# apache/cassandra

Hardware: NVIDIA H100
Metric: compaction MB/s (uncompressed in) (higher is better)
Workload: dtype u8

## Files before the change

cassandra_b200/csrc/codec.cuh:

```cuda
#pragma once
#include "common.cuh"
#include "lz4.cuh"
#include "lz4_chain.cuh"
#include "snappy_chain.cuh"
#include "snappy.cuh"
#include "codec_defs.cuh"
#include "lz4_thread.cuh"
#include "lz4_batch.cuh"

namespace b200c {

__global__ void __launch_bounds__(32) k_compress_chunks(const DevTables* __restrict__ T, int comp, int tab_bytes,
        const uint8_t* __restrict__ in, uint64_t n, int chunk_len, int max_clen,
        uint8_t* __restrict__ slots, int slot_stride, uint32_t* __restrict__ file_len, uint32_t* __restrict__ seg_raw) {
    extern __shared__ __align__(16) uint8_t smem[];
    uint16_t* s_tab = (uint16_t*)smem;
    uint8_t* s_in = smem + tab_bytes;
    const int lane = threadIdx.x;
    const uint64_t chunk = blockIdx.x;
    const uint64_t start = chunk * (uint64_t)chunk_len;
    const int ulen = (int)min((uint64_t)chunk_len, n - start);
    const uint8_t* src = in + start;

    if ((((uintptr_t)src) & 15) == 0) {
// ... 412 lines not shown
}

enum : uint32_t { K1_SKIP = 0xFFFFFFFFu, K1_BAD = 0xFFFFFFFEu, K1_BAD_OFFS = 0xFFFFFFFDu, K1_RAW = 0xFFFFFFFCu };
struct K1Chunk { const uint8_t* src; uint8_t* dst; int clen, ulen; uint64_t slot, ctag; };
__device__ __forceinline__ uint32_t k1_locate(const K1Seg* __restrict__ segs, int nseg, uint64_t t, K1Chunk& k) {
    int lo = 0, hi = nseg - 1;
    while (lo < hi) { int mid = (lo + hi + 1) >> 1; if (segs[mid].first <= t) lo = mid; else hi = mid - 1; }
    const K1Seg& g = segs[lo];
    const uint64_t chunk = g.chunk0 + (t - g.first);
    if (chunk >= g.nchunks) return K1_SKIP;
    const uint64_t off = g.offs[chunk], next = (chunk + 1 < g.nchunks) ? g.offs[chunk + 1] : g.data_len, off0 = g.offs[g.chunk0];
    const uint64_t ustart = chunk * (uint64_t)g.chunk_len;
    k.ctag = ((uint64_t)g.tag << 40) | chunk;
    if (off + 4 > next || next > g.data_len || ustart >= g.data_length || next - off - 4 > (uint64_t)(chunk_max_compressed(COMP_LZ4, g.chunk_len) + g.chunk_len) ||
        off < off0 || next - off0 > g.rec_span) return K1_BAD_OFFS;
    k.clen = (int)(next - off - 4); k.ulen = (int)min((uint64_t)g.chunk_len, g.data_length - ustart);
    k.src = k1_src(g.data, g.tail, g.tail_off, off); k.dst = g.out + ustart;
    k.slot = g.rec0 + (off - off0) / 3 + 2 * (chunk - g.chunk0);
    return k.clen >= g.max_clen ? K1_RAW : 0u;
}
__global__ void __launch_bounds__(128) k_lz4_walk_multi(const K1Seg* __restrict__ segs, int nseg, uint64_t total, uint16_t* __restrict__ rec,
                                                        uint32_t* __restrict__ nseq, ChunkErr* __restrict__ err) {
    const uint64_t t = (uint64_t)blockIdx.x * blockDim.x + threadIdx.x;
    if (t >= total) return;
    K1Chunk k; const uint32_t st = k1_locate(segs, nseg, t, k);
    if (st == K1_SKIP) { nseq[t] = K1_SKIP; return; }
    if (st == K1_BAD_OFFS) { report_chunk_err(err, k.ctag, 2); nseq[t] = K1_BAD_OFFS; return; }
    if (st == K1_RAW) { if (k.clen < k.ulen) { report_chunk_err(err, k.ctag, 2); nseq[t] = K1_BAD; } else nseq[t] = K1_RAW; return; }
    const uint8_t* src = k.src;
    const int plen = (k.clen >= 4) ? (int)((uint32_t)src[0] | ((uint32_t)src[1] << 8) | ((uint32_t)src[2] << 16) | ((uint32_t)src[3] << 24)) : -1;
    const int r = (plen == k.ulen) ? lz4_walk_thread(src + 4, k.clen - 4, k.ulen, rec + k.slot, (k.clen + 4) / 3 + 1) : -1;
    if (r < 0) { report_chunk_err(err, k.ctag, 2); nseq[t] = K1_BAD; } else nseq[t] = (uint32_t)r;
}
enum { K1C_WARPS = 4 };
__global__ void __launch_bounds__(32 * K1C_WARPS) k_lz4_copy_multi(const DevTables* __restrict__ T, const K1Seg* __restrict__ segs, int nseg, uint64_t total,
                                                                   const uint16_t* __restrict__ rec, const uint32_t* __restrict__ nseq, int verify, ChunkErr* __restrict__ err) {
    const int lane = threadIdx.x & 31;
    const uint64_t t = (uint64_t)blockIdx.x * K1C_WARPS + (threadIdx.x >> 5);
    if (t >= total) return;
    const uint32_t ns = nseq[t];
    if (ns == K1_SKIP || ns == K1_BAD_OFFS) return;
    K1Chunk k; (void)k1_locate(segs, nseg, t, k);
    if (verify) {
        const uint32_t crc = warp_crc32(T, T->crc_adv128, k.src, k.clen, lane);
        const uint8_t* s = k.src + k.clen;
        const uint32_t stored = ((uint32_t)s[0] << 24) | ((uint32_t)s[1] << 16) | ((uint32_t)s[2] << 8) | s[3];
        if (crc != stored) { if (lane == 0) report_chunk_err(err, k.ctag, 1); return; }
    }
    if (ns == K1_BAD) return;
    if (ns == K1_RAW) { for (int i = lane; i < k.ulen; i += 32) k.dst[i] = k.src[i]; return; }
    (void)lz4_copy_warp(k.src + 4, k.clen - 4, rec + k.slot, (int)ns, k.dst, lane);
}

}
```

cassandra_b200/csrc/engine.cu:

```cuda
#include "engine.cuh"
#include <algorithm>
#include "scan.cuh"
#include "codec.cuh"
#include <climits>
#include <vector>

using namespace b200c;

namespace b200c {

enum { WSC_IN = 0, WSC_OUT, WSC_SLOTS, WSC_FILELEN, WSC_SEGRAW, WSC_OFFS, WSC_ACC, WSC_ERR, WSC_CHOFFS, WSC_SCAN0, WSC_SCAN1, WSC_SCAN2 };
int raw_chunks_device(b200c_ctx* c, bool ingest, const RawArgs& a);
static int raw_digest(b200c_ctx* c, const uint32_t* seg_raw, const uint64_t* ends, uint64_t nchunks, uint32_t* acc, uint32_t* digest);

static void build_tables(DevTables* t) {
    for (uint32_t i = 0; i < 256; i++) {
        uint32_t c = i;
        for (int k = 0; k < 8; k++) c = (c & 1) ? (0xEDB88320u ^ (c >> 1)) : (c >> 1);
        t->crc_t[0][i] = c;
    }
    for (uint32_t i = 0; i < 256; i++)
        for (int k = 1; k < 4; k++) t->crc_t[k][i] = (t->crc_t[k - 1][i] >> 8) ^ t->crc_t[0][t->crc_t[k - 1][i] & 0xff];
    uint32_t sq = 0x00800000u;
    for (int k = 0; k < 64; k++) { t->xp_pow2[k] = sq; sq = gf2_mulmod(sq, sq); }
// ... 177 lines not shown
    b200c_ctx* c = o.c;
    *out_len = 0; *digest = 0; *d_offs_out = nullptr;
    if (!o.nchunks) return B200C_OK;
    if (o.raw) {
        B200C_TRY(raw_digest(c, o.seg_raw, o.ends, o.nchunks, o.acc, digest));
        B200C_CUDA_TRY(c, cudaStreamSynchronize(c->copy_out));
        *out_len = o.ulen; *d_offs_out = o.d_offs;
        return B200C_OK;
    }
    uint32_t* h32 = &c->h_pinned->os_digest;
    B200C_LAUNCH(c, k_digest, (unsigned)((o.nchunks + 255) / 256), 256, 0, c->d_tables, o.seg_raw, o.d_offs, o.nchunks, o.acc);
    B200C_LAUNCH(c, k_digest_final, 1, 1, 0, c->d_tables, o.d_offs, o.nchunks, o.acc);
    B200C_CUDA_TRY(c, cudaMemcpyAsync(h32, o.acc + 1, 4, cudaMemcpyDeviceToHost, c->stream));
    B200C_TRY(out_stream_drain(o, o.piece - 1));
    B200C_CUDA_TRY(c, cudaStreamSynchronize(c->stream));
    B200C_CUDA_TRY(c, cudaStreamSynchronize(c->copy_out));
    *out_len = o.copied; *digest = h32[0]; *d_offs_out = o.d_offs;
    return B200C_OK;
}

static void k1_plan(b200c_ctx* c) {
    static const int carveout_kb[] = {0, 8, 16, 32, 64, 100, 132, 164, 196, 228};
    const int per_sm = (int)std::max<uint64_t>(1, (uint64_t)c->l2_bytes / K1_L2_BYTES_PER_CHAIN / K1_THREADS / (uint64_t)c->nsm);
    const int block = c->smem_reserved_per_block + K1_STATIC_SMEM;
    int carve = c->smem_per_sm;
    for (int kb : carveout_kb) if (kb * 1024 >= per_sm * block) { carve = std::min(kb * 1024, c->smem_per_sm); break; }
    c->k1_blocks_per_sm = per_sm;
    c->k1_smem = (size_t)std::max(0, (carve / per_sm - block) & ~127);
    for (const void* k : {(const void*)k_decompress_multi_thr, (const void*)k_decompress_chunks_thr}) {
        cudaFuncSetAttribute(k, cudaFuncAttributeMaxDynamicSharedMemorySize, (int)c->k1_smem);
        cudaFuncSetAttribute(k, cudaFuncAttributePreferredSharedMemoryCarveout, 100 * carve / c->smem_per_sm);
    }
}
static unsigned k1_grid(const b200c_ctx* c, uint64_t nthreads) {
    return (unsigned)std::min<uint64_t>((uint64_t)c->k1_blocks_per_sm * (uint64_t)c->nsm, (nthreads + K1_THREADS - 1) / K1_THREADS);
}

int decompress_stream_device(b200c_ctx* c, int comp, const uint8_t* d_data, uint64_t data_len, const uint64_t* d_offs, uint64_t nchunks,
                             int chunk_len, int max_clen, uint64_t data_length, uint8_t* d_out, int verify, ChunkErr* d_err,
                             uint64_t chunk0, uint64_t count, int tag, const uint8_t* tail, uint64_t tail_off) {
    if (chunk0 >= nchunks || count == 0) return B200C_OK;
    const uint64_t end = count > nchunks - chunk0 ? nchunks : chunk0 + count;
    static const int k1_mode = []() { const char* e = getenv("B200C_K1"); return e ? atoi(e) : 1; }();
    if (k1_mode == 1 && comp == COMP_LZ4 && (chunk_len & 7) == 0 && ((uintptr_t)d_out & 7) == 0 && end - chunk0 >= 32768)
        B200C_LAUNCH(c, k_decompress_chunks_thr, k1_grid(c, end - chunk0), K1_THREADS, c->k1_smem, c->d_tables, comp, d_data, data_len, d_offs, nchunks,
                     chunk_len, max_clen, data_length, d_out, verify, d_err, chunk0, end, tag, tail, tail_off);
    else
        B200C_LAUNCH(c, k_decompress_chunks, (unsigned)((end - chunk0 + 1) / 2), 64, 0, c->d_tables, comp, d_data, data_len, d_offs, nchunks,
                     chunk_len, max_clen, data_length, d_out, verify, d_err, chunk0, end, tag, tail, tail_off);
    return B200C_OK;
}

int decompress_multi_device(b200c_ctx* c, K1Seg* segs, int nseg, int verify, ChunkErr* d_err, int ws_slot) {
    uint64_t total = 0;
    for (int i = 0; i < nseg; i++) { segs[i].first = total; segs[i].count = segs[i].nchunks > segs[i].chunk0 ? std::min(segs[i].count, segs[i].nchunks - segs[i].chunk0) : 0; total += segs[i].count; }
    if (!total) return B200C_OK;
    static const int k1_mode = []() { const char* e = getenv("B200C_K1"); return e ? atoi(e) : 1; }();
    uint64_t rec_total = 0;
    for (int i = 0; i < nseg; i++) {
        if (!segs[i].rec_span || segs[i].rec_span > segs[i].data_len) segs[i].rec_span = segs[i].data_len;
        segs[i].rec0 = rec_total; rec_total += segs[i].rec_span / 3 + 2 * segs[i].count + 8;
    }
    K1Seg* d; B200C_TRY(ws_typed(c, ws_slot, (size_t)nseg + 1, &d));
    B200C_CUDA_TRY(c, cudaMemcpyAsync(d, segs, sizeof(K1Seg) * nseg, cudaMemcpyHostToDevice, c->stream));
    if (k1_mode == 2) {
        uint16_t* rec; uint32_t* nseq;
        B200C_TRY(ws_typed(c, WS_K1_REC, (size_t)rec_total + 64, &rec));
        B200C_TRY(ws_typed(c, WS_K1_NSEQ, (size_t)total + 64, &nseq));
        B200C_LAUNCH(c, k_lz4_walk_multi, (unsigned)((total + 127) / 128), 128, 0, d, nseg, total, rec, nseq, d_err);
        static const int copy_blocks = []() { const char* e = getenv("B200C_K1_COPY_BLOCKS"); int v = e ? atoi(e) : 8; return v < 1 ? 1 : (v > 16 ? 16 : v); }();
        static bool attr = false; if (!attr) { cudaFuncSetAttribute(k_lz4_copy_multi, cudaFuncAttributeMaxDynamicSharedMemorySize, 220 * 1024); attr = true; }
        const size_t pad = copy_blocks >= 16 ? 0 : (size_t)(220 * 1024) / copy_blocks;
        B200C_LAUNCH(c, k_lz4_copy_multi, (unsigned)((total + K1C_WARPS - 1) / K1C_WARPS), 32 * K1C_WARPS, pad, c->d_tables, (const K1Seg*)d, nseg, total, (const uint16_t*)rec, (const uint32_t*)nseq, verify, d_err);
        return B200C_OK;
    }
    unsigned long long* next = (unsigned long long*)(d + nseg);
    B200C_CUDA_TRY(c, cudaMemsetAsync(next, 0, sizeof(*next), c->stream));
    B200C_LAUNCH(c, k_decompress_multi_thr, k1_grid(c, total), K1_THREADS, c->k1_smem, c->d_tables, d, nseg, total, verify, d_err, next);
    return B200C_OK;
}

int raw_chunks_device(b200c_ctx* c, bool ingest, const RawArgs& a) {
    if (a.chunk_end <= a.chunk0) return B200C_OK;
    const unsigned grid = (unsigned)std::min<uint64_t>(a.chunk_end - a.chunk0, (uint64_t)c->nsm * 8);
    if (ingest) B200C_LAUNCH(c, k_raw_ingest, grid, RAW_THREADS, 0, c->d_tables, a);
    else B200C_LAUNCH(c, k_raw_checksum, grid, RAW_THREADS, 0, c->d_tables, a);
    return B200C_OK;
}
static int raw_digest(b200c_ctx* c, const uint32_t* seg_raw, const uint64_t* ends, uint64_t nchunks, uint32_t* acc, uint32_t* digest) {
    B200C_LAUNCH(c, k_digest, (unsigned)((nchunks + 255) / 256), 256, 0, c->d_tables, seg_raw, ends, nchunks, acc);
    B200C_LAUNCH(c, k_digest_final, 1, 1, 0, c->d_tables, ends, nchunks, acc);
    uint32_t* h32 = &c->h_pinned->digest;
    B200C_CUDA_TRY(c, cudaMemcpyAsync(h32, acc + 1, 4, cudaMemcpyDeviceToHost, c->stream));
    B200C_CUDA_TRY(c, cudaStreamSynchronize(c->stream));
    *digest = h32[0];
    return B200C_OK;
}
int raw_stream_device(b200c_ctx* c, const uint8_t* d_in, uint64_t n, int chunk_len, uint8_t* d_out, uint64_t* d_crc, uint32_t* digest, int ws_base) {
    const uint64_t nchunks = (n + chunk_len - 1) / chunk_len;
    *digest = 0;
    if (!nchunks) return B200C_OK;
    uint32_t *seg_raw, *acc; uint64_t* ends;
    B200C_TRY(ws_typed(c, ws_base + WSC_SEGRAW, nchunks + 1, &seg_raw));
    B200C_TRY(ws_typed(c, ws_base + WSC_SCAN1, nchunks + 2, &ends));
    B200C_TRY(ws_typed(c, ws_base + WSC_ACC, 4, &acc));
    B200C_CUDA_TRY(c, cudaMemsetAsync(acc, 0, 16, c->stream));
    RawArgs a; memset(&a, 0, sizeof(a));
    a.src = d_in; a.dst = d_out; a.n = n; a.L = chunk_len; a.chunk_end = nchunks; a.crc_out = d_crc; a.seg_raw = seg_raw; a.ends = ends;
    B200C_TRY(raw_chunks_device(c, false, a));
    return raw_digest(c, seg_raw, ends, nchunks, acc, digest);
}

}

extern "C" {

int b200c_abi_version(void) { return B200C_ABI_VERSION; }

int b200c_device_count(void) {
    int n = 0; if (cudaGetDeviceCount(&n) != cudaSuccess) { cudaGetLastError(); return 0; } return n;
}

b200c_ctx* b200c_create(int device, size_t workspace_bytes) {
    int n = b200c_device_count();
    if (device < 0 || device >= n) return nullptr;
    if (cudaSetDevice(device) != cudaSuccess) return nullptr;
    b200c_ctx* c = new b200c_ctx();
    c->device = device;
    if (cudaDeviceGetAttribute(&c->nsm, cudaDevAttrMultiProcessorCount, device) != cudaSuccess || c->nsm <= 0) { delete c; return nullptr; }
    if (cudaDeviceGetAttribute(&c->l2_bytes, cudaDevAttrL2CacheSize, device) != cudaSuccess || c->l2_bytes <= 0) { delete c; return nullptr; }
    if (cudaDeviceGetAttribute(&c->smem_per_sm, cudaDevAttrMaxSharedMemoryPerMultiprocessor, device) != cudaSuccess ||
        cudaDeviceGetAttribute(&c->smem_reserved_per_block, cudaDevAttrReservedSharedMemoryPerBlock, device) != cudaSuccess) { delete c; return nullptr; }
    if (cudaStreamCreateWithFlags(&c->stream, cudaStreamNonBlocking) != cudaSuccess) { delete c; return nullptr; }
    cudaEventCreate(&c->ev0); cudaEventCreate(&c->ev1);
    for (auto& e : c->ev_stage) cudaEventCreate(&e);
    cudaStreamCreateWithFlags(&c->copy_stream, cudaStreamNonBlocking);
    for (auto& e : c->ev_in) cudaEventCreateWithFlags(&e, cudaEventDisableTiming);
    for (auto& e : c->ev_pool) cudaEventCreateWithFlags(&e, cudaEventDisableTiming);
    cudaStreamCreateWithFlags(&c->copy_out, cudaStreamNonBlocking);
    DevTables* h = new DevTables(); build_tables(h);
    if (cudaMalloc(&c->d_tables, sizeof(DevTables)) != cudaSuccess) { delete h; delete c; return nullptr; }
    cudaMemcpy(c->d_tables, h, sizeof(DevTables), cudaMemcpyHostToDevice);
    delete h;
    if (cudaMallocHost((void**)&c->h_pinned, H_PINNED_CAP) != cudaSuccess) { cudaFree(c->d_tables); delete c; return nullptr; }
    cudaFuncSetAttribute(k_compress_chunks, cudaFuncAttributeMaxDynamicSharedMemorySize, 65536 + 65536 + 16);
    cudaFuncSetAttribute(k_compress_chunks_snappy_direct, cudaFuncAttributeMaxDynamicSharedMemorySize, 65536);
    k1_plan(c);
    (void)workspace_bytes;
    return c;
}

void b200c_destroy(b200c_ctx* c) {
    if (!c) return;
    cudaSetDevice(c->device);
    cudaStreamSynchronize(c->stream);
    for (auto& b : c->ws) if (b.p) cudaFree(b.p);
    if (c->d_tables) cudaFree(c->d_tables);
    if (c->h_pinned) cudaFreeHost(c->h_pinned);
    cudaEventDestroy(c->ev0); cudaEventDestroy(c->ev1);
    for (auto& e : c->ev_stage) cudaEventDestroy(e);
    for (auto& e : c->ev_in) cudaEventDestroy(e);
    for (auto& e : c->ev_pool) cudaEventDestroy(e);
    for (auto& e : c->ev_marks) cudaEventDestroy(e);
    if (c->copy_out) cudaStreamDestroy(c->copy_out);
    if (c->copy_stream) cudaStreamDestroy(c->copy_stream);
    cudaStreamDestroy(c->stream);
    delete c;
}

const char* b200c_last_error(b200c_ctx* c) { return c ? c->err.c_str() : "no context (no CUDA device?)"; }

int b200c_host_register(void* p, size_t n) { cudaError_t e = cudaHostRegister(p, n, cudaHostRegisterDefault); if (e != cudaSuccess) { cudaGetLastError(); return B200C_ECUDA; } return B200C_OK; }
int b200c_host_unregister(void* p) { cudaError_t e = cudaHostUnregister(p); if (e != cudaSuccess) { cudaGetLastError(); return B200C_ECUDA; } return B200C_OK; }

int b200c_dev_alloc(b200c_ctx* c, size_t n, void** dptr) {
    if (!c || !dptr) return B200C_EINVAL;
    cudaSetDevice(c->device);
    B200C_CUDA_TRY(c, cudaMalloc(dptr, n + 256));
    return B200C_OK;
}
// ... 194 lines not shown
```

cassandra_b200/csrc/engine.cuh:

```cuda
#pragma once
#include <cstdio>
#include <cstring>
#include <string>
#include <atomic>
#include <chrono>
#include <vector>
#include "../../include/b200c.h"
#include "common.cuh"

namespace b200c {

enum { WS_SLOTS = 160, WS_K5_ENT = 150, WS_K1_REC = 151, WS_K1_NSEQ = 152 };

struct WsBuf { void* p = nullptr; size_t cap = 0; };

enum { MAX_RANGES = 16 };
enum { EV_OUT_PIECE = 0, EV_RANGE = 200, EV_INDEX_FREE = 220, EV_INDEX_READY = 221, EV_UOUT_FREE = 230, EV_POOL = 256 };
struct Pinned;

}

struct b200c_ctx {
    int device = 0;
    int nsm = 0;
    int l2_bytes = 0;
    int smem_per_sm = 0, smem_reserved_per_block = 0;
    int k1_blocks_per_sm = 1; size_t k1_smem = 0;
    cudaStream_t stream = nullptr;
    cudaEvent_t ev0 = nullptr, ev1 = nullptr;
    b200c::DevTables* d_tables = nullptr;
    b200c::WsBuf ws[b200c::WS_SLOTS];
    b200c::Pinned* h_pinned = nullptr;
    std::string err;
    uint64_t launches_call = 0, launches_total = 0;
    double last_ms = 0.0;
    std::atomic<int> cancel{0};
    std::atomic<uint64_t> prog_scanned{0}, prog_total{0};
    std::atomic<int> prog_stage{0}; std::atomic<int> prog_seq{0};
    std::atomic<int> prog_ninputs{0};
    std::atomic<uint64_t> prog_input_pos[B200C_MAX_INPUTS];
    bool timing = false;
    cudaEvent_t ev_stage[8] = {nullptr, nullptr, nullptr, nullptr, nullptr, nullptr, nullptr, nullptr};
    double stage_ms[8] = {0, 0, 0, 0, 0, 0, 0, 0};
    int nstages = 0;
    int k4_attr_set = 0, k4s_attr_set = 0;
    cudaStream_t copy_stream = nullptr;
    cudaEvent_t ev_in[64] = {};
    std::vector<cudaEvent_t> ev_marks;
    cudaEvent_t ev_pool[b200c::EV_POOL] = {};
    cudaStream_t copy_out = nullptr;
};

namespace b200c {

#define B200C_CUDA_TRY(ctx, expr) do { cudaError_t _e = (expr); if (_e != cudaSuccess) { \
    (ctx)->err = std::string(#expr) + ": " + cudaGetErrorString(_e); return B200C_ECUDA; } } while (0)

#define B200C_LAUNCH(ctx, kernel, grid, block, smem, ...) do { \
    kernel<<<(grid), (block), (smem), (ctx)->stream>>>(__VA_ARGS__); \
    (ctx)->launches_call++; (ctx)->launches_total++; \
// ... 88 lines not shown
```

cassandra_b200/csrc/lz4_batch.cuh:

```cuda
#pragma once
#include "lz4_thread.cuh"

namespace b200c {

enum { LZ4B_COOP = 48 };

B200C_HD_NOINLINE int lz4_walk_thread(const uint8_t* __restrict__ src, int n, int cap, uint16_t* __restrict__ rec, int rec_cap) {
    if (n == 0) return cap == 0 ? 0 : -1;
    int ip = 0, op = 0, k = 0;
    for (;;) {
        if (ip >= n || k >= rec_cap) return -1;
        const int tpos = ip;
        const uint32_t token = src[ip++];
        int len = (int)(token >> 4);
        if (len == 15) { uint32_t s; do { if (ip >= n) return -1; s = src[ip++]; len += (int)s; } while (s == 255 && len < (1 << 24)); }
        if (n - ip < len || cap - op < len) return -1;
        ip += len; op += len;
        rec[k++] = (uint16_t)tpos;
        if (ip == n) break;
        if (n - ip < 2) return -1;
        const int offset = (int)src[ip] | ((int)src[ip + 1] << 8); ip += 2;
        if (offset == 0 || offset > op) return -1;
        int ml = (int)(token & 15);
        if (ml == 15) { uint32_t s; do { if (ip >= n) return -1; s = src[ip++]; ml += (int)s; } while (s == 255 && ml < (1 << 24)); }
        ml += LZ4T_MINMATCH;
        if (cap - op < ml) return -1;
        op += ml;
    }
    return op == cap ? k : -1;
}

#if defined(__CUDACC__) || defined(B200C_WARP_EMU)
__device__ __forceinline__ int lz4b_count(int arr, int key, bool le) {
    int pos = 0;
#pragma unroll
    for (int step = 16; step; step >>= 1) {
        const int v = __shfl_sync(FULL_MASK, arr, pos + step - 1);
        if (le ? (v <= key) : (v < key)) pos += step;
    }
    return pos;
}

__device__ __forceinline__ int lz4_copy_warp(const uint8_t* __restrict__ src, int n, const uint16_t* __restrict__ rec, int nseq, uint8_t* dst, int lane) {
    const uint32_t lt_mask = (1u << lane) - 1u;
    int base = 0;
    for (int b0 = 0; b0 < nseq; b0 += 32) {
        const int i = b0 + lane;
        int lit = 0, ml = 0, off = 0, ls = 0;
        if (i < nseq) {
            int q = (int)rec[i];
            const uint32_t t = src[q++];
            lit = (int)(t >> 4);
            if (lit == 15) { uint32_t s; do { s = src[q++]; lit += (int)s; } while (s == 255); }
            ls = q; q += lit;
            if (q < n) {
                off = (int)src[q] | ((int)src[q + 1] << 8); q += 2;
                ml = (int)(t & 15);
                if (ml == 15) { uint32_t s; do { s = src[q++]; ml += (int)s; } while (s == 255); }
                ml += LZ4T_MINMATCH;
            }
        }
        const int tot = lit + ml;
        int incl = tot;
#pragma unroll
        for (int d = 1; d < 32; d <<= 1) { const int t2 = __shfl_sync(FULL_MASK, incl, lane - d); if (lane >= d) incl += t2; }
        const int my_op = base + incl - tot, mop = my_op + lit;
        base += __shfl_sync(FULL_MASK, incl, 31);
        if (lit <= LZ4B_COOP) for (int k = 0; k < lit; k++) dst[my_op + k] = src[ls + k];
        for (uint32_t big = __ballot_sync(FULL_MASK, lit > LZ4B_COOP); big; big &= big - 1) {
            const int l = __ffs(big) - 1;
            const int bs = __shfl_sync(FULL_MASK, ls, l), bo = __shfl_sync(FULL_MASK, my_op, l), bn = __shfl_sync(FULL_MASK, lit, l);
            for (int k = lane; k < bn; k += 32) dst[bo + k] = src[bs + k];
        }
        __syncwarp();
        const int s = mop - off, e = (off < ml) ? mop : s + ml;
        const int k_lo = lz4b_count(mop + ml, s, true);
        const int k_hi = lz4b_count(mop, e, false);
        const uint32_t upto_hi = k_hi >= 32 ? FULL_MASK : ((1u << k_hi) - 1u);
        const uint32_t dep = upto_hi & ~((1u << k_lo) - 1u) & lt_mask;
        bool pending = ml > 0;
        for (;;) {
            const uint32_t pm = __ballot_sync(FULL_MASK, pending);
            if (!pm) break;
            const bool can = pending && !(pm & dep);
            if (can && ml <= LZ4B_COOP) {
                if (off >= ml) for (int k = 0; k < ml; k++) dst[mop + k] = dst[s + k];
                else for (int k = 0; k < ml; k++) dst[mop + k] = dst[s + k % off];
            }
            for (uint32_t big = __ballot_sync(FULL_MASK, can && ml > LZ4B_COOP); big; big &= big - 1) {
                const int l = __ffs(big) - 1;
                const int bs = __shfl_sync(FULL_MASK, s, l), bo = __shfl_sync(FULL_MASK, mop, l), bn = __shfl_sync(FULL_MASK, ml, l), bf = __shfl_sync(FULL_MASK, off, l);
                for (int k = lane; k < bn; k += 32) dst[bo + k] = dst[bs + (k < bf ? k : k % bf)];
            }
            if (can) pending = false;
            __syncwarp();
        }
    }
    return base;
}
#endif

}
```

cassandra_b200/csrc/compact.cu:

```cuda
#include "engine.cuh"
#include "scan.cuh"
#include "codec_defs.cuh"
#include "partition.cuh"
#include "partition_tile.cuh"
#include "meta.cuh"
#include "index_walk.cuh"
#include <climits>
#include <vector>
#include <algorithm>
#include <cmath>

using namespace b200c;

namespace b200c {

int compress_stream_device(b200c_ctx* c, int comp, const uint8_t* d_in, uint64_t n, int chunk_len, int max_clen,
                           uint8_t* d_out, uint64_t out_cap, uint64_t* d_offs, uint64_t* out_len, uint32_t* digest, int ws_base);
int compress_slots_device(b200c_ctx* c, int comp, const uint8_t* d_in, uint64_t n, int chunk_len, int max_clen,
                          uint8_t* slots, int stride, uint32_t* file_len, uint32_t* seg_raw);
int pack_digest_device(b200c_ctx* c, const uint8_t* slots, int stride, const uint32_t* file_len, const uint32_t* seg_raw, uint64_t nchunks,
                       uint8_t* d_out, uint64_t out_cap, uint64_t* d_offs, uint64_t* out_len, uint32_t* digest, int ws_base);
int decompress_stream_device(b200c_ctx* c, int comp, const uint8_t* d_data, uint64_t data_len, const uint64_t* d_offs, uint64_t nchunks,
                             int chunk_len, int max_clen, uint64_t data_length, uint8_t* d_out, int verify, ChunkErr* d_err, uint64_t chunk0, uint64_t count, int tag,
                             const uint8_t* tail, uint64_t tail_off);
// ... 713 lines not shown
    MCell* merged = WIDE ? merged_local : cells + (size_t)tid * ncols_s;
    DT open_dt[ST_MAXM];
    StatAcc acc; acc.init(sP->now, a.td);
    for (uint32_t t = tid; t < np; t += ST_THREADS) {
        const uint32_t j = j0 + s_order[t];
        const uint64_t cj = a.op_first[j]; const uint32_t m = (uint32_t)(a.op_first[j + 1] - cj);
        const uint32_t m_uni = min((uint32_t)ST_MAXM, __reduce_max_sync(__activemask(), m));
        uint8_t *dout, *iout; uint64_t dcap, dposv; uint32_t nbf, ipf, ixs_cap;
        if (!k4_prologue<true>(a, j, dout, dcap, dposv, iout, nbf, ipf, ixs_cap)) continue;
        PartOut out{0, 0, 0, 0, 0}; PartStats st{0, 0}; int e = 0;
        if (m > (uint32_t)ST_MAXM || cj - c0 + m > (uint64_t)ST_CUR_CAP) e = PERR_UNSUPPORTED;
        else process_partition<true>(*sP, xl, a.contrib, cj, m, a.upos, a.pbase, a.kp, a.klen, a.tok, dout, dcap, dposv, iout, nbf, ipf, ixs_cap, curs + (cj - c0), open_dt, merged, out, st, e,
                                     a.sg ? &acc : nullptr, m_uni);
        k4_epilogue<true>(a, j, cj, out, st, e);
    }
    if (a.sg) stat_flush_warp(a.sg, acc);
}

__global__ void __launch_bounds__(256) k_bounds(const uint64_t* __restrict__ contrib, const uint64_t* __restrict__ op_first, uint64_t nparts,
                                                const uint64_t* __restrict__ upos, const uint64_t* __restrict__ pbase, uint64_t* __restrict__ bound,
                                                uint32_t column_index_size, uint32_t* __restrict__ icap, uint32_t* __restrict__ insz, uint8_t* __restrict__ big) {
    uint64_t j = (uint64_t)blockIdx.x * blockDim.x + threadIdx.x;
    if (j >= nparts) return;
    uint64_t sum = 0;
    for (uint64_t c = op_first[j]; c < op_first[j + 1]; c++) { uint64_t e = contrib[c]; uint64_t g = pbase[(e >> 56) & 0x7F] + (e & 0xFFFFFFFFFFull); sum += upos[g + 1] - upos[g]; }
    uint64_t b = (sum + (sum >> 2) + 32 + 15) & ~15ull;
    bound[j] = b;
    insz[j] = (uint32_t)min(sum, (uint64_t)0xFFFFFFFFull);
    big[j] = (sum > (uint64_t)ST_MAXP || op_first[j + 1] - op_first[j] > (uint64_t)ST_MAXM) ? 1 : 0;
    uint64_t nb_max = b / column_index_size + 2;
    icap[j] = (b > column_index_size && nb_max < (1u << 23)) ? (uint32_t)(IXS_HEAD + nb_max * IXS_BLOCK_STRIDE) : 0u;
}

__global__ void __launch_bounds__(256) k_gather(uint64_t nparts, const uint64_t* __restrict__ dsize, const uint64_t* __restrict__ dpos, const uint64_t* __restrict__ bpos,
                                                const uint8_t* __restrict__ ovf, const uint8_t* __restrict__ scratch, uint8_t* __restrict__ uout) {
    uint64_t j = (uint64_t)blockIdx.x * 8 + (threadIdx.x >> 5);
    if (j >= nparts) return;
    uint64_t n = dsize[j];
    if (!n || ovf[j]) return;
    const uint8_t* s = scratch + bpos[j]; uint8_t* d = uout + dpos[j];
    int lane = threadIdx.x & 31;
    for (uint64_t i = lane; i < n; i += 32) d[i] = s[i];
}

__global__ void __launch_bounds__(256) k_index_simple(const CParams* __restrict__ Pp, uint64_t nparts, const uint64_t* __restrict__ contrib, const uint64_t* __restrict__ op_first,
        const uint64_t* __restrict__ upos, const uint64_t* __restrict__ pbase, const uint64_t* __restrict__ dsize, const uint64_t* __restrict__ dpos,
        const uint32_t* __restrict__ nblk, const uint8_t* __restrict__ ovf, const uint32_t* __restrict__ ihead, const uint64_t* __restrict__ ipos, uint8_t* __restrict__ iout) {
    uint64_t j = (uint64_t)blockIdx.x * blockDim.x + threadIdx.x;
    if (j >= nparts || !dsize[j] || nblk[j] > 1 || ovf[j]) return;
    uint64_t e = contrib[op_first[j]]; uint64_t g = pbase[(e >> 56) & 0x7F] + (e & 0xFFFFFFFFFFull);
    const uint8_t* k = Pp->U + upos[g];
    uint32_t n = ihead[j];
    Sink<true> s{iout + ipos[j], 0, true, ~0ull};
    s.copy(k, n); s.vint(dpos[j]); s.u8(0);
}

__global__ void __launch_bounds__(128) k_index_promoted(const CParams* __restrict__ Pp, uint64_t nparts, const uint64_t* __restrict__ contrib, const uint64_t* __restrict__ op_first,
        const uint64_t* __restrict__ upos, const uint64_t* __restrict__ pbase, const uint64_t* __restrict__ dsize, const uint64_t* __restrict__ dpos,
        const uint32_t* __restrict__ nblk, const uint8_t* __restrict__ ovf, const uint32_t* __restrict__ ihead, const uint32_t* __restrict__ ipay, const uint64_t* __restrict__ ipos,
        const uint64_t* __restrict__ ioff, const uint32_t* __restrict__ icap, const uint8_t* __restrict__ iscr, uint8_t* __restrict__ iout) {
    uint64_t j = (uint64_t)blockIdx.x * blockDim.x + threadIdx.x;
    if (j >= nparts || !dsize[j] || nblk[j] <= 1 || ovf[j]) return;
    uint64_t e = contrib[op_first[j]]; uint64_t g = pbase[(e >> 56) & 0x7F] + (e & 0xFFFFFFFFFFull);
    const uint8_t* k = Pp->U + upos[g];
    const uint8_t* slot = iscr + ioff[j];
    const uint32_t nb_max = (icap[j] - IXS_HEAD) / IXS_BLOCK_STRIDE, nb = nblk[j], n = ihead[j];
    DT pd; pd.mfda = ((const int64_t*)slot)[0]; pd.ldt = ((const int64_t*)slot)[1];
    const uint32_t pdsz = dt_is_live(pd) ? 1u : 12u, hdr_len = (uint32_t)((const int64_t*)slot)[2];
    const uint32_t infos = ipay[j] - vint_size(hdr_len) - pdsz - vint_size(nb) - 4 * nb;
    Sink<true> s{iout + ipos[j], 0, true, ~0ull};
    s.copy(k, n); s.vint(dpos[j]); s.vint(ipay[j]);
    s.vint(hdr_len); write_partition_dt(s, pd); s.vint(nb);
    s.copy(slot + IXS_HEAD + 4 * (size_t)nb_max, infos); s.copy(slot + IXS_HEAD, 4 * nb);
}

// ... 824 lines not shown
        if (!staged) return launch_k4(1);
        uint64_t *d_inpos, *d_tscan; uint32_t *d_mark, *d_tstart; unsigned long long* d_nbig = (unsigned long long*)(d_stats + 1);
        B200C_TRY(ws_typed(c, WS_INPOS, nparts + 2, &d_inpos));
        B200C_TRY(ws_typed(c, WS_TMARK, nparts + 2, &d_mark));
        B200C_TRY(ws_typed(c, WS_TSCAN, nparts + 2, &d_tscan));
        B200C_TRY(ws_typed(c, WS_TSTART, nparts + 2, &d_tstart));
        B200C_TRY(exclusive_scan<uint32_t>(c, d_insz, nparts, d_inpos, WS_SCANA, 0));
        B200C_CUDA_TRY(c, cudaMemsetAsync(d_nbig, 0, 8, st));
        B200C_LAUNCH(c, k_tile_marks, (unsigned)((nparts + 255) / 256), 256, 0, nparts, d_inpos, d_opfirst, d_big, d_mark, d_nbig);
        B200C_TRY(exclusive_scan<uint32_t>(c, d_mark, nparts, d_tscan, WS_SCANA, 0));
        B200C_LAUNCH(c, k_tile_starts, (unsigned)((nparts + 1 + 255) / 256), 256, 0, nparts, d_mark, d_tscan, d_tstart);
        B200C_CUDA_TRY(c, cudaMemcpyAsync(&P->ntiles, d_tscan + nparts, 8, cudaMemcpyDeviceToHost, st));
        B200C_CUDA_TRY(c, cudaMemcpyAsync(&P->nbig, d_nbig, 8, cudaMemcpyDeviceToHost, st));
        B200C_CUDA_TRY(c, cudaStreamSynchronize(st));
        const bool wide = m->ncolumns > K4_SMEM_COLS;
        const size_t smem_st = (size_t)ST_HEAD + ST_STAGE_CAP + (size_t)ST_CUR_CAP * sizeof(CurS) + (wide ? 0 : (size_t)ST_THREADS * hp.mcols * sizeof(MCell)) + 16;
        if (c->k4s_attr_set != (int)smem_st) { k4_staged_attr<false>(smem_st); k4_staged_attr<true>(smem_st); c->k4s_attr_set = (int)smem_st; }
        ka.mode = 1; ka.only_big = nullptr;
        B200C_TRY(wide ? k4_staged<true>(c, ka, P->ntiles, smem_st, d_tstart, d_big) : k4_staged<false>(c, ka, P->ntiles, smem_st, d_tstart, d_big));
        if (P->nbig) { ka.only_big = d_big; B200C_TRY(launch_k4(1)); ka.only_big = nullptr; }
        return B200C_OK;
    }
    int emit(int r) {
        mark(4);
        if (raw_out && to_host_stream && r >= 2) B200C_CUDA_TRY(c, cudaStreamWaitEvent(st, c->ev_pool[EV_UOUT_FREE + (r & 1)], 0));
        B200C_TRY(ws_typed(c, (r & 1) ? WS_UOUT2 : WS_UOUT, tail_len + ulen_out + 64, &UOUT));
        if (r) B200C_CUDA_TRY(c, cudaStreamWaitEvent(st, c->ev_pool[EV_INDEX_FREE], 0));
        B200C_TRY(ws_typed(c, WS_IOUT, ilen_out + 64, &IOUT));
        if (tail_len) B200C_CUDA_TRY(c, cudaMemcpyAsync(UOUT, tail_ptr, tail_len, cudaMemcpyDeviceToDevice, st));
        uint8_t* const ubias = (uint8_t*)((uintptr_t)UOUT + tail_len - ubase_total);
        if (!nparts || !ulen_out) return B200C_OK;
        ka.dbase = ubias; ka.iout = IOUT; ka.doff = nullptr; ka.dcapv = nullptr;
        if (two_pass) return launch_k4(2);
        B200C_LAUNCH(c, k_gather, (unsigned)((nparts + 7) / 8), 256, 0, nparts, d_dsize, d_dpos, d_bpos, d_ovf, SCRATCH, ubias);
        B200C_LAUNCH(c, k_index_simple, (unsigned)((nparts + 255) / 256), 256, 0, dP, nparts, d_contrib, d_opfirst, d_upos, d_pbase, d_dsize, d_dpos, d_nblk, d_ovf, d_ihead, d_ipos, IOUT);
        B200C_LAUNCH(c, k_index_promoted, (unsigned)((nparts + 127) / 128), 128, 0, dP, nparts, d_contrib, d_opfirst, d_upos, d_pbase, d_dsize, d_dpos, d_nblk, d_ovf, d_ihead, d_ipay, d_ipos,
                     d_ioff, d_icap, ISCR, IOUT);
        return launch_k4(3);
    }
    int meta() {
        const uint64_t ns = (written_total + P->written + meta_interval - 1) / meta_interval - (written_total + meta_interval - 1) / meta_interval;
        uint32_t *d_samplej, *d_esize; uint64_t* d_epos;
        B200C_TRY(ws_typed(c, WS_META_SAMPLE, ns + 1, &d_samplej));
        B200C_TRY(ws_typed(c, WS_META_ESIZE, ns + 1, &d_esize));
        B200C_TRY(ws_typed(c, WS_META_EPOS, ns + 2, &d_epos));
        MetaArgs ma; memset(&ma, 0, sizeof(ma));
        ma.P = dP; ma.contrib = d_contrib; ma.op_first = d_opfirst; ma.upos = d_upos; ma.pbase = d_pbase; ma.dsize = d_dsize; ma.ipos = d_ipos; ma.ihead = d_ihead;
        ma.ccount = d_ccount; ma.wrank = d_wrank; ma.nparts = nparts; ma.index_base = ilen_total; ma.written_base = written_total; ma.sg = d_sg;
        ma.bloom = d_bloom; ma.bloom_bits = bloom_words * 64; ma.bloom_k = m->bloom_hash_count; ma.interval = meta_interval; ma.sample_j = d_samplej;
        ma.first_key = d_mkeys; ma.last_key = d_mkeys + 65536;
        B200C_LAUNCH(c, k_meta_keys, (unsigned)((nparts + 255) / 256), 256, 0, ma);
        if (ns && res->outputs[0].summary) {
            B200C_LAUNCH(c, k_summary_sizes, (unsigned)((ns + 255) / 256), 256, 0, ma, ns, d_esize);
            B200C_TRY(exclusive_scan<uint32_t>(c, d_esize, ns, d_epos, WS_SCANA, 0));
            B200C_CUDA_TRY(c, cudaMemcpyAsync(&P->summary_len, d_epos + ns, 8, cudaMemcpyDeviceToHost, st));
            B200C_CUDA_TRY(c, cudaStreamSynchronize(st));
            B200C_TRY(ws_grow_keep<uint8_t>(c, WS_META_SUMENT, sument_bound + P->summary_len + 64, sument_bound, &d_sument));
            B200C_TRY(ws_grow_keep<uint64_t>(c, WS_META_SUMOFF, samples_total + ns + 2, samples_total, &d_sumoff));
            B200C_LAUNCH(c, k_summary_emit, (unsigned)((ns + 255) / 256), 256, 0, ma, ns, d_epos, d_sument, d_sumoff);
            B200C_LAUNCH(c, k_meta_advance, 1, 1, 0, d_sg, ns, d_epos);
            sument_bound += P->summary_len; samples_total += ns;
        }
        written_total += P->written;
        return B200C_OK;
    }
    int k5_stream(int r) {
        mark(5);
// ... 284 lines not shown
```

Before: 35770.

## Decompress LZ4 chunks in a per-warp shared-memory window and copy out vectorized

Replaces the multi-segment LZ4 copy kernel with one that stages each compressed record into a per-warp shared-memory window, decodes in place into that window, then writes the result to global memory with 16-byte vector stores. Literal and match copies now use word-sized loads and stores, and a 'tight' path serializes literal copies when the output could overrun the not-yet-consumed input in the shared window. The goal is to turn scattered byte-wise global accesses into shared-memory work plus coalesced global writes. The cost is a large dynamic shared-memory allocation per block, which limits occupancy, plus extra syncs. Records too large for the window are flagged as errors unless stored raw.

```diff
diff --git a/cassandra_b200/csrc/codec.cuh b/cassandra_b200/csrc/codec.cuh
--- a/cassandra_b200/csrc/codec.cuh
+++ b/cassandra_b200/csrc/codec.cuh
@@ -468,24 +468,63 @@
     const int r = (plen == k.ulen) ? lz4_walk_thread(src + 4, k.clen - 4, k.ulen, rec + k.slot, (k.clen + 4) / 3 + 1) : -1;
     if (r < 0) { report_chunk_err(err, k.ctag, 2); nseq[t] = K1_BAD; } else nseq[t] = (uint32_t)r;
 }
-enum { K1C_WARPS = 4 };
-__global__ void __launch_bounds__(32 * K1C_WARPS) k_lz4_copy_multi(const DevTables* __restrict__ T, const K1Seg* __restrict__ segs, int nseg, uint64_t total,
-                                                                   const uint16_t* __restrict__ rec, const uint32_t* __restrict__ nseq, int verify, ChunkErr* __restrict__ err) {
-    const int lane = threadIdx.x & 31;
-    const uint64_t t = (uint64_t)blockIdx.x * K1C_WARPS + (threadIdx.x >> 5);
+enum { K1S_MAX_WARPS = 4 };
+__device__ __forceinline__ void k1s_store(const uint8_t* w, int o, int len, uint8_t* dst, int lane) {
+    if (((uintptr_t)dst & 15) == 0) {
+        const int nv = len >> 4;
+        if ((o & 15) == 0) {
+            for (int i = lane; i < nv; i += 32) ((uint4*)dst)[i] = ((const uint4*)(w + o))[i];
+        } else {
+            const uint32_t* q0 = (const uint32_t*)(w + (o & ~3)); const int sh = (o & 3) * 8;
+            for (int i = lane; i < nv; i += 32) {
+                const uint32_t* q = q0 + 4 * i;
+                const uint32_t a = q[0], b = q[1], c = q[2], d = q[3], e = q[4];
+                ((uint4*)dst)[i] = make_uint4(__funnelshift_r(a, b, sh), __funnelshift_r(b, c, sh), __funnelshift_r(c, d, sh), __funnelshift_r(d, e, sh));
+            }
+        }
+        for (int i = (nv << 4) + lane; i < len; i += 32) dst[i] = w[o + i];
+    } else {
+        for (int i = lane; i < len; i += 32) dst[i] = w[o + i];
+    }
+}
+__global__ void __launch_bounds__(32 * K1S_MAX_WARPS, 3) k_lz4_copy_smem(const DevTables* __restrict__ T, const K1Seg* __restrict__ segs, int nseg, uint64_t total,
+        const uint16_t* __restrict__ rec, const uint32_t* __restrict__ nseq, int verify, ChunkErr* __restrict__ err, int win) {
+    extern __shared__ __align__(16) uint8_t s_k1s[];
+    const int lane = threadIdx.x & 31, wid = threadIdx.x >> 5;
+    const uint64_t t = (uint64_t)blockIdx.x * (blockDim.x >> 5) + wid;
     if (t >= total) return;
     const uint32_t ns = nseq[t];
     if (ns == K1_SKIP || ns == K1_BAD_OFFS) return;
     K1Chunk k; (void)k1_locate(segs, nseg, t, k);
+    uint8_t* w = s_k1s + (size_t)wid * win;
+    const int rlen = k.clen + 4;
+    if (rlen + 48 > win) {
+        if (verify) {
+            const uint32_t crc = warp_crc32(T, T->crc_adv128, k.src, k.clen, lane);
+            const uint8_t* s = k.src + k.clen;
+            if (crc != (((uint32_t)s[0] << 24) | ((uint32_t)s[1] << 16) | ((uint32_t)s[2] << 8) | s[3])) { if (lane == 0) report_chunk_err(err, k.ctag, 1); return; }
+        }
+        if (ns == K1_RAW) for (int i = lane; i < k.ulen; i += 32) k.dst[i] = k.src[i];
+        else if (ns != K1_BAD && lane == 0) report_chunk_err(err, k.ctag, 2);
+        return;
+    }
+    const int mis = (int)((uintptr_t)k.src & 15);
+    const int at = k1s_record_at(win, rlen, mis);
+    {
+        const uint4* g = (const uint4*)(k.src - mis); uint4* s4 = (uint4*)(w + at - mis);
+        const int nv = (mis + rlen + 15) >> 4;
+        for (int i = lane; i < nv; i += 32) s4[i] = __ldg(g + i);
+    }
+    __syncwarp();
     if (verify) {
-        const uint32_t crc = warp_crc32(T, T->crc_adv128, k.src, k.clen, lane);
-        const uint8_t* s = k.src + k.clen;
-        const uint32_t stored = ((uint32_t)s[0] << 24) | ((uint32_t)s[1] << 16) | ((uint32_t)s[2] << 8) | s[3];
-        if (crc != stored) { if (lane == 0) report_chunk_err(err, k.ctag, 1); return; }
+        const uint32_t crc = warp_crc32(T, T->crc_adv128, w + at, k.clen, lane);
+        const uint8_t* s = w + at + k.clen;
+        if (crc != (((uint32_t)s[0] << 24) | ((uint32_t)s[1] << 16) | ((uint32_t)s[2] << 8) | s[3])) { if (lane == 0) report_chunk_err(err, k.ctag, 1); return; }
     }
     if (ns == K1_BAD) return;
-    if (ns == K1_RAW) { for (int i = lane; i < k.ulen; i += 32) k.dst[i] = k.src[i]; return; }
-    (void)lz4_copy_warp(k.src + 4, k.clen - 4, rec + k.slot, (int)ns, k.dst, lane);
-}
-
-}
+    int o = at;
+    if (ns != K1_RAW) { (void)lz4_copy_warp(w + at + 4, k.clen - 4, rec + k.slot, (int)ns, w, lane); __syncwarp(); o = 0; }
+    k1s_store(w, o, k.ulen, k.dst, lane);
+}
+
+}
diff --git a/cassandra_b200/csrc/engine.cu b/cassandra_b200/csrc/engine.cu
--- a/cassandra_b200/csrc/engine.cu
+++ b/cassandra_b200/csrc/engine.cu
@@ -233,6 +233,10 @@
         cudaFuncSetAttribute(k, cudaFuncAttributePreferredSharedMemoryCarveout, 100 * carve / c->smem_per_sm);
     }
 }
+static void k1_copy_plan(b200c_ctx* c) {
+    cudaFuncSetAttribute(k_lz4_copy_smem, cudaFuncAttributeMaxDynamicSharedMemorySize, c->smem_per_block_optin);
+    cudaFuncSetAttribute(k_lz4_copy_smem, cudaFuncAttributePreferredSharedMemoryCarveout, 100);
+}
 static unsigned k1_grid(const b200c_ctx* c, uint64_t nthreads) {
     return (unsigned)std::min<uint64_t>((uint64_t)c->k1_blocks_per_sm * (uint64_t)c->nsm, (nthreads + K1_THREADS - 1) / K1_THREADS);
 }
@@ -257,10 +261,11 @@
     for (int i = 0; i < nseg; i++) { segs[i].first = total; segs[i].count = segs[i].nchunks > segs[i].chunk0 ? std::min(segs[i].count, segs[i].nchunks - segs[i].chunk0) : 0; total += segs[i].count; }
     if (!total) return B200C_OK;
     static const int k1_mode = []() { const char* e = getenv("B200C_K1"); return e ? atoi(e) : 1; }();
-    uint64_t rec_total = 0;
+    uint64_t rec_total = 0; int max_chunk = 0;
     for (int i = 0; i < nseg; i++) {
         if (!segs[i].rec_span || segs[i].rec_span > segs[i].data_len) segs[i].rec_span = segs[i].data_len;
         segs[i].rec0 = rec_total; rec_total += segs[i].rec_span / 3 + 2 * segs[i].count + 8;
+        if (segs[i].count) max_chunk = std::max(max_chunk, segs[i].chunk_len);
     }
     K1Seg* d; B200C_TRY(ws_typed(c, ws_slot, (size_t)nseg + 1, &d));
     B200C_CUDA_TRY(c, cudaMemcpyAsync(d, segs, sizeof(K1Seg) * nseg, cudaMemcpyHostToDevice, c->stream));
@@ -269,10 +274,10 @@
         B200C_TRY(ws_typed(c, WS_K1_REC, (size_t)rec_total + 64, &rec));
         B200C_TRY(ws_typed(c, WS_K1_NSEQ, (size_t)total + 64, &nseq));
         B200C_LAUNCH(c, k_lz4_walk_multi, (unsigned)((total + 127) / 128), 128, 0, d, nseg, total, rec, nseq, d_err);
-        static const int copy_blocks = []() { const char* e = getenv("B200C_K1_COPY_BLOCKS"); int v = e ? atoi(e) : 8; return v < 1 ? 1 : (v > 16 ? 16 : v); }();
-        static bool attr = false; if (!attr) { cudaFuncSetAttribute(k_lz4_copy_multi, cudaFuncAttributeMaxDynamicSharedMemorySize, 220 * 1024); attr = true; }
-        const size_t pad = copy_blocks >= 16 ? 0 : (size_t)(220 * 1024) / copy_blocks;
-        B200C_LAUNCH(c, k_lz4_copy_multi, (unsigned)((total + K1C_WARPS - 1) / K1C_WARPS), 32 * K1C_WARPS, pad, c->d_tables, (const K1Seg*)d, nseg, total, (const uint16_t*)rec, (const uint32_t*)nseq, verify, d_err);
+        const int win = k1s_window(max_chunk);
+        const int warps = std::max(1, std::min<int>(K1S_MAX_WARPS, c->smem_per_block_optin / win));
+        B200C_LAUNCH(c, k_lz4_copy_smem, (unsigned)((total + warps - 1) / warps), 32 * warps, (size_t)warps * win, c->d_tables, (const K1Seg*)d, nseg, total,
+                     (const uint16_t*)rec, (const uint32_t*)nseq, verify, d_err, win);
         return B200C_OK;
     }
     unsigned long long* next = (unsigned long long*)(d + nseg);
@@ -331,7 +336,8 @@
     if (cudaDeviceGetAttribute(&c->nsm, cudaDevAttrMultiProcessorCount, device) != cudaSuccess || c->nsm <= 0) { delete c; return nullptr; }
     if (cudaDeviceGetAttribute(&c->l2_bytes, cudaDevAttrL2CacheSize, device) != cudaSuccess || c->l2_bytes <= 0) { delete c; return nullptr; }
     if (cudaDeviceGetAttribute(&c->smem_per_sm, cudaDevAttrMaxSharedMemoryPerMultiprocessor, device) != cudaSuccess ||
-        cudaDeviceGetAttribute(&c->smem_reserved_per_block, cudaDevAttrReservedSharedMemoryPerBlock, device) != cudaSuccess) { delete c; return nullptr; }
+        cudaDeviceGetAttribute(&c->smem_reserved_per_block, cudaDevAttrReservedSharedMemoryPerBlock, device) != cudaSuccess ||
+        cudaDeviceGetAttribute(&c->smem_per_block_optin, cudaDevAttrMaxSharedMemoryPerBlockOptin, device) != cudaSuccess) { delete c; return nullptr; }
     if (cudaStreamCreateWithFlags(&c->stream, cudaStreamNonBlocking) != cudaSuccess) { delete c; return nullptr; }
     cudaEventCreate(&c->ev0); cudaEventCreate(&c->ev1);
     for (auto& e : c->ev_stage) cudaEventCreate(&e);
@@ -347,6 +353,7 @@
     cudaFuncSetAttribute(k_compress_chunks, cudaFuncAttributeMaxDynamicSharedMemorySize, 65536 + 65536 + 16);
     cudaFuncSetAttribute(k_compress_chunks_snappy_direct, cudaFuncAttributeMaxDynamicSharedMemorySize, 65536);
     k1_plan(c);
+    k1_copy_plan(c);
     (void)workspace_bytes;
     return c;
 }
diff --git a/cassandra_b200/csrc/engine.cuh b/cassandra_b200/csrc/engine.cuh
--- a/cassandra_b200/csrc/engine.cuh
+++ b/cassandra_b200/csrc/engine.cuh
@@ -26,6 +26,7 @@
     int l2_bytes = 0;
     int smem_per_sm = 0, smem_reserved_per_block = 0;
     int k1_blocks_per_sm = 1; size_t k1_smem = 0;
+    int smem_per_block_optin = 0;
     cudaStream_t stream = nullptr;
     cudaEvent_t ev0 = nullptr, ev1 = nullptr;
     b200c::DevTables* d_tables = nullptr;
diff --git a/cassandra_b200/csrc/lz4_batch.cuh b/cassandra_b200/csrc/lz4_batch.cuh
--- a/cassandra_b200/csrc/lz4_batch.cuh
+++ b/cassandra_b200/csrc/lz4_batch.cuh
@@ -4,6 +4,10 @@
 namespace b200c {
 
 enum { LZ4B_COOP = 48 };
+
+enum { K1S_SLACK = 2048 };
+B200C_HD int k1s_window(int chunk_len) { return chunk_len + K1S_SLACK; }
+B200C_HD int k1s_record_at(int win, int rlen, int mis) { return ((win - 32 - rlen) & ~15) + mis; }
 
 B200C_HD_NOINLINE int lz4_walk_thread(const uint8_t* __restrict__ src, int n, int cap, uint16_t* __restrict__ rec, int rec_cap) {
     if (n == 0) return cap == 0 ? 0 : -1;
@@ -41,7 +45,32 @@
     return pos;
 }
 
-__device__ __forceinline__ int lz4_copy_warp(const uint8_t* __restrict__ src, int n, const uint16_t* __restrict__ rec, int nseq, uint8_t* dst, int lane) {
+__device__ __forceinline__ uint32_t lz4b_ld32(const uint8_t* p) {
+    const uintptr_t a = (uintptr_t)p; const uint32_t* q = (const uint32_t*)(a & ~(uintptr_t)3);
+    return (uint32_t)((((uint64_t)q[1] << 32) | q[0]) >> ((a & 3) * 8));
+}
+__device__ __forceinline__ void lz4b_copy(uint8_t* d, const uint8_t* s, int len) {
+    int k = 0;
+    int head = (int)((4 - ((uintptr_t)d & 3)) & 3); if (head > len) head = len;
+    for (; k < head; k++) d[k] = s[k];
+    for (; k + 4 <= len; k += 4) *(uint32_t*)(d + k) = lz4b_ld32(s + k);
+    for (; k < len; k++) d[k] = s[k];
+}
+__device__ __forceinline__ void lz4b_copy_coop(uint8_t* d, const uint8_t* s, int len, bool sync, int lane) {
+    int head = (int)((4 - ((uintptr_t)d & 3)) & 3); if (head > len) head = len;
+    if (lane < head) d[lane] = s[lane];
+    if (sync) __syncwarp();
+    const int nw = (len - head) >> 2;
+    for (int w0 = 0; w0 < nw; w0 += 32) {
+        const int k = head + 4 * (w0 + lane);
+        if (w0 + lane < nw) *(uint32_t*)(d + k) = lz4b_ld32(s + k);
+        if (sync) __syncwarp();
+    }
+    const int t = head + 4 * nw + lane;
+    if (t < len) d[t] = s[t];
+}
+
+__device__ __forceinline__ int lz4_copy_warp(const uint8_t* src, int n, const uint16_t* __restrict__ rec, int nseq, uint8_t* dst, int lane) {
     const uint32_t lt_mask = (1u << lane) - 1u;
     int base = 0;
     for (int b0 = 0; b0 < nseq; b0 += 32) {
@@ -65,13 +94,24 @@
 #pragma unroll
         for (int d = 1; d < 32; d <<= 1) { const int t2 = __shfl_sync(FULL_MASK, incl, lane - d); if (lane >= d) incl += t2; }
         const int my_op = base + incl - tot, mop = my_op + lit;
-        base += __shfl_sync(FULL_MASK, incl, 31);
-        if (lit <= LZ4B_COOP) for (int k = 0; k < lit; k++) dst[my_op + k] = src[ls + k];
-        for (uint32_t big = __ballot_sync(FULL_MASK, lit > LZ4B_COOP); big; big &= big - 1) {
-            const int l = __ffs(big) - 1;
-            const int bs = __shfl_sync(FULL_MASK, ls, l), bo = __shfl_sync(FULL_MASK, my_op, l), bn = __shfl_sync(FULL_MASK, lit, l);
-            for (int k = lane; k < bn; k += 32) dst[bo + k] = src[bs + k];
+        const int step_end = base + __shfl_sync(FULL_MASK, incl, 31);
+        const bool tight = (uintptr_t)(dst + step_end) > (uintptr_t)(src + rec[b0]);
+        if (!tight) {
+            if (lit <= LZ4B_COOP) lz4b_copy(dst + my_op, src + ls, lit);
+            for (uint32_t big = __ballot_sync(FULL_MASK, lit > LZ4B_COOP); big; big &= big - 1) {
+                const int l = __ffs(big) - 1;
+                const int bs = __shfl_sync(FULL_MASK, ls, l), bo = __shfl_sync(FULL_MASK, my_op, l), bn = __shfl_sync(FULL_MASK, lit, l);
+                lz4b_copy_coop(dst + bo, src + bs, bn, false, lane);
+            }
+        } else {
+            for (uint32_t any = __ballot_sync(FULL_MASK, lit > 0); any; any &= any - 1) {
+                const int l = __ffs(any) - 1;
+                const int bs = __shfl_sync(FULL_MASK, ls, l), bo = __shfl_sync(FULL_MASK, my_op, l), bn = __shfl_sync(FULL_MASK, lit, l);
+                lz4b_copy_coop(dst + bo, src + bs, bn, true, lane);
+                __syncwarp();
+            }
         }
+        base = step_end;
         __syncwarp();
         const int s = mop - off, e = (off < ml) ? mop : s + ml;
         const int k_lo = lz4b_count(mop + ml, s, true);
@@ -84,13 +124,16 @@
             if (!pm) break;
             const bool can = pending && !(pm & dep);
             if (can && ml <= LZ4B_COOP) {
-                if (off >= ml) for (int k = 0; k < ml; k++) dst[mop + k] = dst[s + k];
-                else for (int k = 0; k < ml; k++) dst[mop + k] = dst[s + k % off];
+                uint8_t* d = dst + mop;
+                int k = 0, dist = off;
+                if (off < 4) { const int e4 = off == 3 ? 3 : 4 - off; for (; k < e4 && k < ml; k++) d[k] = d[k - off]; dist = off == 3 ? 6 : 4; }
+                lz4b_copy(d + k, d + k - dist, ml - k);
             }
             for (uint32_t big = __ballot_sync(FULL_MASK, can && ml > LZ4B_COOP); big; big &= big - 1) {
                 const int l = __ffs(big) - 1;
                 const int bs = __shfl_sync(FULL_MASK, s, l), bo = __shfl_sync(FULL_MASK, mop, l), bn = __shfl_sync(FULL_MASK, ml, l), bf = __shfl_sync(FULL_MASK, off, l);
-                for (int k = lane; k < bn; k += 32) dst[bo + k] = dst[bs + (k < bf ? k : k % bf)];
+                if (bf >= 128) lz4b_copy_coop(dst + bo, dst + bs, bn, true, lane);
+                else for (int k = lane; k < bn; k += 32) dst[bo + k] = dst[bs + (k < bf ? k : k % bf)];
             }
             if (can) pending = false;
             __syncwarp();
```

Result: no change. 35780, median of 6 (+0.0%).

## Gather output bytes per warp across 32 partitions as one contiguous span

Applied to the files above, without the earlier changes.

Each warp of the gather kernel now covers 32 consecutive partitions instead of one. It stages their destination and source offsets in shared memory and walks the combined output span with an 8-way unrolled byte loop, looking up the owning partition for each byte. This is meant to keep lanes busy when partitions are small, where one warp per partition leaves most lanes idle and launches many tiny blocks. It relies on dpos being contiguous, so that dpos[j+1]-dpos[j] equals dsize. It also reads dpos at index nparts, and overflowed partitions are skipped with a sentinel, which may break if those assumptions do not hold.

```diff
diff --git a/cassandra_b200/csrc/compact.cu b/cassandra_b200/csrc/compact.cu
--- a/cassandra_b200/csrc/compact.cu
+++ b/cassandra_b200/csrc/compact.cu
@@ -769,15 +769,34 @@
     icap[j] = (b > column_index_size && nb_max < (1u << 23)) ? (uint32_t)(IXS_HEAD + nb_max * IXS_BLOCK_STRIDE) : 0u;
 }
 
-__global__ void __launch_bounds__(256) k_gather(uint64_t nparts, const uint64_t* __restrict__ dsize, const uint64_t* __restrict__ dpos, const uint64_t* __restrict__ bpos,
+__global__ void __launch_bounds__(256) k_gather(uint64_t nparts, const uint64_t* __restrict__ dpos, const uint64_t* __restrict__ bpos,
                                                 const uint8_t* __restrict__ ovf, const uint8_t* __restrict__ scratch, uint8_t* __restrict__ uout) {
-    uint64_t j = (uint64_t)blockIdx.x * 8 + (threadIdx.x >> 5);
-    if (j >= nparts) return;
-    uint64_t n = dsize[j];
-    if (!n || ovf[j]) return;
-    const uint8_t* s = scratch + bpos[j]; uint8_t* d = uout + dpos[j];
-    int lane = threadIdx.x & 31;
-    for (uint64_t i = lane; i < n; i += 32) d[i] = s[i];
+    enum { UNROLL = 8 };
+    __shared__ uint64_t s_dp[8][33], s_bp[8][32];
+    const int w = threadIdx.x >> 5, lane = threadIdx.x & 31;
+    const uint64_t j0 = ((uint64_t)blockIdx.x * 8 + w) * 32;
+    if (j0 >= nparts) return;
+    const uint32_t cnt = (uint32_t)min((uint64_t)32, nparts - j0);
+    if (lane < cnt) { s_dp[w][lane] = dpos[j0 + lane]; s_bp[w][lane] = ovf[j0 + lane] ? ~0ull : bpos[j0 + lane]; }
+    if (lane == 0) s_dp[w][cnt] = dpos[j0 + cnt];
+    __syncwarp();
+    const uint64_t d0 = s_dp[w][0], n = s_dp[w][cnt] - d0;
+    uint32_t p = 0;
+    for (uint64_t i = lane; i < n; i += 32 * UNROLL) {
+        uint8_t v[UNROLL]; uint64_t at[UNROLL];
+#pragma unroll
+        for (int u = 0; u < UNROLL; u++) {
+            at[u] = ~0ull;
+            const uint64_t x = d0 + i + 32 * u;
+            if (i + 32 * u >= n) continue;
+            while (s_dp[w][p + 1] <= x) p++;
+            const uint64_t b = s_bp[w][p];
+            if (b == ~0ull) continue;
+            v[u] = scratch[b + (x - s_dp[w][p])]; at[u] = x;
+        }
+#pragma unroll
+        for (int u = 0; u < UNROLL; u++) if (at[u] != ~0ull) uout[at[u]] = v[u];
+    }
 }
 
 __global__ void __launch_bounds__(256) k_index_simple(const CParams* __restrict__ Pp, uint64_t nparts, const uint64_t* __restrict__ contrib, const uint64_t* __restrict__ op_first,
@@ -1668,7 +1687,7 @@
         if (!nparts || !ulen_out) return B200C_OK;
         ka.dbase = ubias; ka.iout = IOUT; ka.doff = nullptr; ka.dcapv = nullptr;
         if (two_pass) return launch_k4(2);
-        B200C_LAUNCH(c, k_gather, (unsigned)((nparts + 7) / 8), 256, 0, nparts, d_dsize, d_dpos, d_bpos, d_ovf, SCRATCH, ubias);
+        B200C_LAUNCH(c, k_gather, (unsigned)((nparts + 255) / 256), 256, 0, nparts, d_dpos, d_bpos, d_ovf, SCRATCH, ubias);
         B200C_LAUNCH(c, k_index_simple, (unsigned)((nparts + 255) / 256), 256, 0, dP, nparts, d_contrib, d_opfirst, d_upos, d_pbase, d_dsize, d_dpos, d_nblk, d_ovf, d_ihead, d_ipos, IOUT);
         B200C_LAUNCH(c, k_index_promoted, (unsigned)((nparts + 127) / 128), 128, 0, dP, nparts, d_contrib, d_opfirst, d_upos, d_pbase, d_dsize, d_dpos, d_nblk, d_ovf, d_ihead, d_ipay, d_ipos,
                      d_ioff, d_icap, ISCR, IOUT);
```

New measurement: 35670 before, 36070 after, median of 6. +1.1%, better.
